# seung-lab/crackle

Measured on AMD Instinct MI355X. Metric: voxels/s encode+decode, 1024x1024x512 uint32; bit-exact .ckl bytes, higher is better.
Workload: dtype u32

## Files before the change

crackle_amd/csrc/ckl_encode.hip:

```cpp
#include "ckl_common.hpp"
#include "ckl_runs.hpp"
#include "ckl_trail.hpp"
#include "ckl_pins_dev.hpp"

#include <algorithm>
#include <atomic>
#include <chrono>
#include <functional>
#include <memory>
#include <mutex>

namespace ckl {

using namespace dev;

template <typename LABEL>
__global__ void __launch_bounds__(kBlock) k_stats(const LABEL* __restrict__ labels, uint64_t voxels, unsigned long long* __restrict__ out ) {
	__shared__ unsigned long long s_max[kWaves], s_pairs[kWaves];
	unsigned long long mx = 0, pairs = 0;
	const uint64_t stride = static_cast<uint64_t>(gridDim.x) * kBlock;
	for (uint64_t i = static_cast<uint64_t>(blockIdx.x) * kBlock + threadIdx.x; i < voxels; i += stride) {
		const LABEL v = labels[i];
		if (static_cast<unsigned long long>(v) > mx) mx = v;
		if (i > 0) pairs += (labels[i - 1] == v);
// ... 1290 lines not shown
	std::vector<uint32_t> code_len;
	uint64_t total = 0;
	bool any_chain = false;
};

inline size_t trail_walk_lds(uint32_t max_special) { return (static_cast<size_t>(max_special) + 256) * 16 + 1024; }

void crack_pass(
	ckl_encoder& e, int64_t sx, int64_t sy, int64_t sz, bool permissible,
	int markov_order, bool hist_only, const std::vector<uint8_t>* model_in,
	std::vector<uint32_t>* hist_out, std::vector<uint8_t>* model_out, CrackResult* result,
	const std::function<void()>& overlap = std::function<void()>(), bool reuse_trail = false
) {
	hipStream_t s = e.stream;
	const uint32_t ns = static_cast<uint32_t>(sz);
	const uint64_t nverts = static_cast<uint64_t>(sx + 1) * (sy + 1);
	e.d_slice_err.ensure(ns);
	const bool prezeroed = e.trail_zeroed && !reuse_trail;
	e.trail_zeroed = false;
	if (prezeroed) CKL_HIP(hipStreamWaitEvent(s, e.ev_prezero, 0));
	if (!reuse_trail && !prezeroed) CKL_HIP(hipMemsetAsync(e.d_slice_err.p, 0, ns * sizeof(uint32_t), s));
	const uint64_t interior = static_cast<uint64_t>(sx > 0 ? sx - 1 : 0) * sy + static_cast<uint64_t>(sx) * (sy > 0 ? sy - 1 : 0);

	std::vector<uint64_t> cbase(ns), sbase(ns), kbase(ns);
	std::vector<uint32_t> ccap(ns), scap(ns), kcap(ns), max_steps(ns);
	std::vector<uint64_t> nbase(ns), cobase(ns), ibase(ns);
	std::vector<uint32_t> ncap(ns), cocap(ns), icap(ns);
	uint64_t ctot = 0, stot = 0, ktot = 0, ntot = 0, cotot = 0, itot = 0;
	uint32_t max_ncap = 0, max_cocap = 0, max_icap = 0, max_special = 0;
	bool any = false;
	for (uint32_t zi = 0; zi < ns; zi++) {
		const uint64_t differ = static_cast<uint64_t>(e.count_v[zi]) + e.count_h[zi];
		const uint64_t E = permissible ? interior - differ : differ;
		any = any || E > 0;
		const uint64_t cc = ((7 * E + 16 + 15) / 16) * 16;
		if (cc > 0xFFFFFFF0ull) throw Error(CKL_ERR_RUNTIME, "crackle_amd: slice has too many crack edges");
		cbase[zi] = ctot; ccap[zi] = static_cast<uint32_t>(cc); ctot += cc;
		max_steps[zi] = static_cast<uint32_t>(E + 1);
		const uint64_t nc = ((static_cast<uint64_t>(e.count_special[zi]) + e.count_corner[zi] + 16) / 16) * 16;
		if (nc >= (1ull << 28)) throw Error(CKL_ERR_RUNTIME, "crackle_amd: slice has too many crack vertices");
		nbase[zi] = ntot; ncap[zi] = static_cast<uint32_t>(nc); ntot += nc;
		cobase[zi] = cotot; cocap[zi] = e.count_corner[zi]; cotot += e.count_corner[zi];
		const uint64_t ic = 7 * nc + 16;
		ibase[zi] = itot; icap[zi] = static_cast<uint32_t>(ic); itot += ic;
		sbase[zi] = stot; scap[zi] = static_cast<uint32_t>(2 * nc + 4); stot += 2 * nc + 4;
		kbase[zi] = ktot; kcap[zi] = static_cast<uint32_t>(nc); ktot += nc;
		max_ncap = std::max<uint32_t>(max_ncap, ncap[zi]);
		max_cocap = std::max<uint32_t>(max_cocap, cocap[zi]);
		max_icap = std::max<uint32_t>(max_icap, icap[zi]);
		max_special = std::max<uint32_t>(max_special, e.count_special[zi]);
	}
	if (result) result->any_chain = any;
	if (g_ht && g_ht->on) {
		uint32_t over = 0;
		for (uint32_t zi = 0; zi < ns; zi++) over += e.count_special[zi] > 3584u;
		fprintf(stderr, "[ckl trail nodes] max special %u, slices above 3584: %u of %u\n", max_special, over, ns);
	}
	HT_MARK("c:caps");
	UploadPacker tables;
	tables.add(e.d_cbase, cbase); tables.add(e.d_ccap, ccap);
	tables.add(e.d_sbase, sbase); tables.add(e.d_scap, scap);
	tables.add(e.d_kbase, kbase); tables.add(e.d_kcap, kcap);
	e.d_cp.ensure(ctot); e.d_fcode.ensure(ctot);
	if (markov_order) e.d_dcode.ensure(ctot);
	e.d_stack_node.ensure(stot); e.d_stack_code.ensure(stot);
	e.d_chain_node.ensure(ktot); e.d_chain_off.ensure(ktot); e.d_chain_clen.ensure(ktot);
	e.d_chain_order.ensure(ktot); e.d_chain_dst.ensure(ktot); e.d_chain_vstart.ensure(ktot);
	e.d_n_chains.ensure(ns); e.d_n_raw.ensure(ns); e.d_n_valid.ensure(ns);
	e.d_payload_len.ensure(ns); e.d_boc_len.ensure(ns);

	const int xw = byte_width(static_cast<uint64_t>(sx) + 1), yw = byte_width(static_cast<uint64_t>(sy) + 1);
	std::vector<uint64_t> pbase(ns), bbase(ns);
	uint64_t ptot = 0, btot = 0;
	for (uint32_t zi = 0; zi < ns; zi++) {
		const uint64_t ncodes = ccap[zi];
		const uint64_t pbytes = markov_order ? (3ull * ncodes + 2 + 7) / 8 : (ncodes + 3) / 4;
		pbase[zi] = ptot; ptot += ((pbytes + 8 + 3) / 4) * 4;
		const uint64_t bbytes = 4 + yw + static_cast<uint64_t>(kcap[zi]) * (yw + 2 * xw);
		bbase[zi] = btot; btot += bbytes;
	}
	tables.add(e.d_pbase, pbase); tables.add(e.d_bbase, bbase);
	tables.add(e.t_nbase, nbase); tables.add(e.t_ncap, ncap);
	tables.add(e.t_cobase, cobase); tables.add(e.t_cocap, cocap);
	tables.add(e.t_ibase, ibase); tables.add(e.t_icap, icap);
	tables.add(e.t_max_steps, max_steps);
	tables.commit(e.d_crack_tables, s, e.uploads_by_kernel ? &e.tables_staging : nullptr);
	HT_MARK("c:tables");
	e.d_payload.ensure(ptot + 8); e.d_boc.ensure(btot + 8);
	e.codes_capacity = ptot + btot;
	if (markov_order) CKL_HIP(hipMemsetAsync(e.d_payload.p, 0, ptot + 8, s));

	FinishArgs fa;
	fa.sx = static_cast<int>(sx); fa.sy = static_cast<int>(sy); fa.xw = xw; fa.yw = yw;
	fa.markov = markov_order ? 1u : 0u;
	fa.cbase = e.d_cbase.p; fa.kbase = e.d_kbase.p;
	fa.n_chains = e.d_n_chains.p; fa.n_raw = e.d_n_raw.p; fa.n_valid = e.d_n_valid.p;
	fa.cp = e.d_cp.p; fa.chain_node = e.d_chain_node.p; fa.chain_off = e.d_chain_off.p; fa.chain_clen = e.d_chain_clen.p;
	fa.chain_order = e.d_chain_order.p; fa.chain_dst = e.d_chain_dst.p; fa.chain_vstart = e.d_chain_vstart.p;
	fa.fcode = e.d_fcode.p; fa.dcode = e.d_dcode.p;
	fa.pbase = e.d_pbase.p; fa.payload = e.d_payload.p; fa.bbase = e.d_bbase.p; fa.boc = e.d_boc.p;
	fa.payload_len = e.d_payload_len.p; fa.boc_len = e.d_boc_len.p;

	unsigned long long* ta_dbg = nullptr;
	size_t trail_lds_used = 0;
	DevBuf<unsigned long long> d_tdbg;
	CKL_HIP(hipEventRecord(e.evk0, s));
	if (!reuse_trail) {
		e.t_counters.ensure(7 * static_cast<size_t>(ns));
		if (!prezeroed) CKL_HIP(hipMemsetAsync(e.t_counters.p, 0, 7 * static_cast<size_t>(ns) * sizeof(uint32_t), s));
		e.t_node_vertex.ensure(ntot); e.t_node_adj.ensure(ntot + 16); e.t_vert2node.ensure(nverts * ns);
		e.t_corner_vertex.ensure(cotot);
		e.t_dart_end.ensure(4 * ntot); e.t_dart_len.ensure(4 * ntot); e.t_dart_minv.ensure(4 * ntot); e.t_dart_minpos.ensure(4 * ntot);
		e.t_dart_codes.ensure(4 * ntot); e.t_dart_inline.ensure(4 * ntot);
		e.t_parent.ensure(ntot); e.t_compmin.ensure(ntot); e.t_starts.ensure(ntot);
		const uint32_t start_words = static_cast<uint32_t>((nverts + 31) / 32);
		e.t_start_bits.ensure(static_cast<size_t>(start_words) * ns);
		if (!prezeroed) CKL_HIP(hipMemsetAsync(e.t_start_bits.p, 0, static_cast<size_t>(start_words) * ns * sizeof(uint32_t), s));
		e.t_items.ensure(itot); e.t_item_off.ensure(itot); e.t_chain_item0.ensure(ktot);
		e.t_events.ensure(itot); e.t_chain_ev0.ensure(ktot); e.t_ev_lnd.ensure(itot); e.t_ev_item.ensure(itot);

		TrailArgs ta;
		ta.adjm = e.d_adjm.p; ta.adjm_stride = e.adjm_stride; ta.mtx2 = e.mtx2; ta.tiles_x = e.tiles_x; ta.tiles_y = e.tiles_y;
		ta.planeV = e.d_planes.p; ta.planeH = e.d_planes.p + e.plane_words * ns; ta.row_words = e.row_words; ta.plane_words = e.plane_words;
		ta.sx = static_cast<uint32_t>(sx); ta.sy = static_cast<uint32_t>(sy); ta.inv = e.graph_permissible ? 0xFFFFFFFFu : 0u;
		ta.sxe = static_cast<uint32_t>(sx + 1); ta.sye = static_cast<uint32_t>(sy + 1); ta.nverts = static_cast<uint32_t>(nverts);
		ta.max_steps = e.t_max_steps.p;
		ta.nbase = e.t_nbase.p; ta.ncap = e.t_ncap.p;
		ta.n_nodes = e.t_counters.p; ta.n_corners = e.t_counters.p + 2 * ns;
		ta.n_starts = e.t_counters.p + 3 * ns; ta.n_items = e.t_counters.p + 4 * ns;
		ta.node_vertex = e.t_node_vertex.p; ta.node_adj = e.t_node_adj.p; ta.vert2node = e.t_vert2node.p;
		ta.cobase = e.t_cobase.p; ta.cocap = e.t_cocap.p; ta.corner_vertex = e.t_corner_vertex.p;
		ta.dart_end = e.t_dart_end.p; ta.dart_len = e.t_dart_len.p; ta.dart_minv = e.t_dart_minv.p; ta.dart_minpos = e.t_dart_minpos.p;
		ta.dart_codes = e.t_dart_codes.p; ta.dart_inline = e.t_dart_inline.p;
		ta.parent = e.t_parent.p; ta.compmin = e.t_compmin.p;
		ta.start_bits = e.t_start_bits.p; ta.start_words = start_words; ta.starts = e.t_starts.p;
		ta.ibase = e.t_ibase.p; ta.icap = e.t_icap.p; ta.items = e.t_items.p; ta.item_off = e.t_item_off.p;
		ta.sbase = e.d_sbase.p; ta.scap = e.d_scap.p; ta.stack_node = e.d_stack_node.p; ta.stack_item = e.d_stack_code.p;
		ta.kbase = e.d_kbase.p; ta.kcap = e.d_kcap.p;
		ta.chain_node = e.d_chain_node.p; ta.chain_item0 = e.t_chain_item0.p; ta.chain_off = e.d_chain_off.p; ta.chain_clen = e.d_chain_clen.p;
		ta.n_chains = e.d_n_chains.p; ta.n_raw = e.d_n_raw.p; ta.n_valid = e.d_n_valid.p;
		ta.cbase = e.d_cbase.p; ta.ccap = e.d_ccap.p; ta.cp = e.d_cp.p; ta.slice_err = e.d_slice_err.p;

		e.last_trail_slices = ns;
		ta.events = e.t_events.p; ta.n_events = e.t_counters.p + 5 * ns; ta.seg_len_sum = e.t_counters.p + 6 * ns; ta.chain_ev0 = e.t_chain_ev0.p; ta.ev_lnd = e.t_ev_lnd.p; ta.ev_item = e.t_ev_item.p;
		ta.dbg = nullptr;
		{ const char* env = getenv("CKL_TRAIL_WALK"); ta.walk_plain = (env && !strcmp(env, "plain")) ? 1u : 0u; ta.walk_no_regs = (env && !strcmp(env, "lds")) ? 1u : 0u; }
		{ const char* env = getenv("CKL_TRAIL_WALK_STACK"); ta.walk_stack_cap = env ? static_cast<uint32_t>(std::max(1, atoi(env))) : 0xFFFFFFFFu; }
		if (kTuning && getenv("CKL_TRAIL_DIAG")) { d_tdbg.ensure(16); CKL_HIP(hipMemsetAsync(d_tdbg.p, 0, 128, s)); ta.dbg = d_tdbg.p; ta_dbg = d_tdbg.p; }
		ta.graph_blocks = e.graph_blocks; ta.blk_special = e.t_blk_special.p; ta.blk_corner = e.t_blk_corner.p;
		int max_lds = 0;
		CKL_HIP(hipDeviceGetAttribute(&max_lds, hipDeviceAttributeMaxSharedMemoryPerBlock, e.device));
		const size_t budget = static_cast<size_t>(max_lds > 1024 ? max_lds - 1024 : 0);
		const uint32_t dart_blocks = (4 * max_ncap + kWalkChunk * kWaves - 1) / (kWalkChunk * kWaves);
		size_t clds = (static_cast<size_t>(max_special) + 1024) * 4;
		if (const char* env = getenv("CKL_TRAIL_LDS")) clds = static_cast<size_t>(std::max(0, atoi(env)));
		clds = (std::min(budget, std::max<size_t>(clds, 1024)) / 16) * 16;
		CKL_HIP(hipFuncSetAttribute(reinterpret_cast<const void*>(&k_trail_components), hipFuncAttributeMaxDynamicSharedMemorySize, static_cast<int>(clds)));
		size_t lds = trail_walk_lds(max_special);
		if (const char* env = getenv("CKL_TRAIL_LDS")) lds = static_cast<size_t>(std::max(0, atoi(env)));
		lds = std::min(budget, std::max<size_t>(lds, 4096));
		lds = (lds / 16) * 16;
		CKL_HIP(hipFuncSetAttribute(reinterpret_cast<const void*>(&k_trail_walk), hipFuncAttributeMaxDynamicSharedMemorySize, static_cast<int>(lds)));
		trail_lds_used = lds;
		HT_MARK("c:setup");

		ta.z0 = 0;
		fa.z0 = 0;
		if (any) {
			hipLaunchKernelGGL(k_trail_nodes, dim3(e.graph_blocks, ns), dim3(kBlock), 0, s, ta);
			hipLaunchKernelGGL(k_trail_segments, dim3(dart_blocks, ns), dim3(kBlock), 0, s, ta);
			if (max_cocap) hipLaunchKernelGGL(k_trail_loops, dim3((max_cocap + kBlock - 1) / kBlock, ns), dim3(kBlock), 0, s, ta);
			hipLaunchKernelGGL(k_trail_components, dim3(ns), dim3(kCompBlock), clds, s, ta, static_cast<uint32_t>(clds));
		}
		CKL_HIP(hipEventRecord(e.evd0, s));
		hipLaunchKernelGGL(k_trail_walk, dim3(ns), dim3(kWave), lds, s, ta, static_cast<uint32_t>(lds));
		CKL_HIP(hipEventRecord(e.evd1, s));
		hipLaunchKernelGGL(k_trail_items, dim3(ns), dim3(kItemsBlock), 0, s, ta);
		hipLaunchKernelGGL(k_trail_offsets, dim3(ns), dim3(kBlock), 0, s, ta);
		hipLaunchKernelGGL(k_trail_expand, dim3((max_icap + kExpandChunk * kWaves - 1) / (kExpandChunk * kWaves), ns), dim3(kBlock), 0, s, ta);
		hipLaunchKernelGGL(k_finish, dim3(ns), dim3(kFinishBlock), 0, s, fa);
	}
	CKL_HIP(hipEventRecord(e.evk1, s));
	HT_MARK("c:enqueue");
	if (kTuning && getenv("CKL_TRAIL_DIAG")) {
		std::vector<uint32_t> c = download(e.t_counters.p, 5 * static_cast<size_t>(ns), s);
		double m[5] = { 0 };
		for (int k = 0; k < 5; k++) for (uint32_t zi = 0; zi < ns; zi++) m[k] += static_cast<double>(c[static_cast<size_t>(k) * ns + zi]) / ns;
		double sp = 0, co = 0;
		for (uint32_t zi = 0; zi < ns; zi++) { sp += static_cast<double>(e.count_special[zi]) / ns; co += static_cast<double>(e.count_corner[zi]) / ns; }
		if (ta_dbg) {
			std::vector<unsigned long long> g = download(ta_dbg, 16, s);
			if (g[11]) fprintf(stderr, "[ckl trail diag, k_trail_walk] mean cycles per slice: table fill=%.0f fill + walk=%.0f\n", static_cast<double>(g[6]) / g[11], static_cast<double>(g[7]) / g[11]);
			if (g[11]) fprintf(stderr, "[ckl trail diag, k_trail_walk] slices=%llu iterations/slice=%.0f cycles/iteration=%.0f clock=%.2f GHz (cycles / 100 MHz ticks)\n",
				g[11], static_cast<double>(g[8]) / g[11], g[8] ? static_cast<double>(g[9]) / g[8] : 0.0, g[10] ? static_cast<double>(g[9]) / (g[10] * 10.0) : 0.0);
			fprintf(stderr, "[ckl trail diag, k_trail_components, mean cycles per slice] union=%.0f component minima=%.0f starts/splits=%.0f bitmap scan=%.0f\n",
				static_cast<double>(g[12]) / ns, static_cast<double>(g[13]) / ns, static_cast<double>(g[14]) / ns, static_cast<double>(g[15]) / ns);
			fprintf(stderr, "[ckl trail diag, k_trail_segments] waves=%llu iterations/wave mean=%.1f max=%llu cycles/wave mean=%.0f max=%llu cycles/iteration=%.0f active lanes/iteration=%.1f\n",
				g[4], g[4] ? static_cast<double>(g[0]) / g[4] : 0.0, g[1], g[4] ? static_cast<double>(g[2]) / g[4] : 0.0, g[3],
				g[0] ? static_cast<double>(g[2]) / g[0] : 0.0, g[0] ? static_cast<double>(g[5]) / g[0] : 0.0);
		}
		fprintf(stderr, "[ckl trail diag] max degree-1/3/4 vertices of a slice=%u, k_trail_walk LDS=%zu bytes\n", max_special, trail_lds_used);
		fprintf(stderr, "[ckl trail diag, mean per slice] degree-1/3/4 vertices=%.0f corners=%.0f nodes=%.0f starts=%.0f items=%.0f\n", sp, co, m[0], m[3], m[4]);
	}

	const bool early_tail = !markov_order && result != nullptr;
	auto enqueue_tail = [&]() {
		e.d_out_off.ensure(ns);
		e.d_code_report.ensure(static_cast<size_t>(ns) + 3);
		e.d_codes_out.ensure(e.codes_capacity + 8);
		hipLaunchKernelGGL(k_code_offsets, dim3(1), dim3(kBlock), 0, s, e.d_boc_len.p, e.d_payload_len.p, e.d_slice_err.p, ns, e.d_out_off.p, e.d_code_report.p);
		hipLaunchKernelGGL(k_gather_codes, dim3(ns), dim3(kBlock), 0, s, e.d_boc.p, e.d_bbase.p, e.d_boc_len.p,
			e.d_payload.p, e.d_pbase.p, e.d_payload_len.p, e.d_out_off.p, e.d_codes_out.p);
	};
	if (early_tail) enqueue_tail();
	if (overlap) overlap();
	HT_MARK("c:overlap");


	if (markov_order) {
		std::vector<uint8_t> model;
		if (model_in) {
			model = *model_in;
		}
		else {
			const size_t rows = static_cast<size_t>(1) << (2 * markov_order);
			e.d_hist.ensure(rows * 4);
			CKL_HIP(hipMemsetAsync(e.d_hist.p, 0, rows * 4 * sizeof(uint32_t), s));
			const uint32_t hist_lds = (rows * 4 <= 16384) ? static_cast<uint32_t>(rows * 4) : 0u;
			if (hist_lds * 4 > 48 * 1024) CKL_HIP(hipFuncSetAttribute(reinterpret_cast<const void*>(&k_markov_hist), hipFuncAttributeMaxDynamicSharedMemorySize, static_cast<int>(hist_lds * 4)));
			hipLaunchKernelGGL(k_markov_hist, dim3(ns), dim3(kBlock), hist_lds * sizeof(uint32_t), s, e.d_dcode.p, e.d_cbase.p, e.d_n_valid.p, markov_order, e.d_hist.p, hist_lds);
			std::vector<uint32_t> hist = download(e.d_hist.p, rows * 4, s);
			if (hist_out) *hist_out = hist;
			if (hist_only) {
				std::vector<uint32_t> errs = download(e.d_slice_err.p, ns, s);
				for (uint32_t zi = 0; zi < ns; zi++) if (errs[zi]) throw Error(CKL_ERR_RUNTIME, "crackle_amd: crack walk scratch overflow on z=" + std::to_string(zi));
				return;
			}
			model = markov_stats_to_model(hist.data(), rows);
		}
		if (model_out) *model_out = model;
		upload(e.d_model, model, s);
		hipLaunchKernelGGL(k_markov_pack, dim3(ns), dim3(kBlock), 0, s, e.d_dcode.p, e.d_cbase.p, e.d_n_valid.p, markov_order,
			e.d_model.p, e.d_pbase.p, e.d_payload.p, e.d_payload_len.p);
	}
	if (!result) { CKL_HIP(hipStreamSynchronize(s)); return; }

	if (!early_tail) enqueue_tail();
	HT_MARK("c:finish_enq");
	std::vector<uint32_t> report = download(e.d_code_report.p, static_cast<size_t>(ns) + 3, s);
	HT_MARK("c:finish_wait");
	if (report[ns + 2]) {
		std::vector<uint32_t> errs = download(e.d_slice_err.p, ns, s);
		for (uint32_t zi = 0; zi < ns; zi++) {
			if (errs[zi]) throw Error(CKL_ERR_RUNTIME, "crackle_amd: crack walk scratch overflow on z=" + std::to_string(zi));
		}
	}
	result->code_len.assign(report.begin(), report.begin() + ns);
	const uint64_t otot = static_cast<uint64_t>(report[ns]) | (static_cast<uint64_t>(report[ns + 1]) << 32);
	result->total = otot;
}

struct FlatResult {
	std::vector<uint32_t> ncomp;
	std::vector<uint32_t> crcs;
	uint64_t total = 0;
};

void ensure_geom_table(ckl_encoder& e, uint64_t sxy) {
	if (e.g_table_pixels == sxy && e.d_G.p) return;
	hipStream_t s = e.stream2;
	const uint32_t npx = static_cast<uint32_t>(sxy);
	const uint32_t B = 1024, nblk = npx / B + 1;
	std::vector<uint32_t> g_base(B), blk_g(nblk), blk_x(nblk);
	const uint32_t X = gf_xpow(32);
	g_base[0] = 0;
	for (uint32_t i = 1; i < B; i++) g_base[i] = gf_mul(X, g_base[i - 1] ^ 0x80000000u);
	const uint32_t gB = gf_mul(X, g_base[B - 1] ^ 0x80000000u);
	const uint32_t XB = gf_xpow(32ull * B);
	blk_g[0] = 0; blk_x[0] = 0x80000000u;
	for (uint32_t k = 1; k < nblk; k++) {
		blk_g[k] = blk_g[k - 1] ^ gf_mul(blk_x[k - 1], gB);
		blk_x[k] = gf_mul(blk_x[k - 1], XB);
	}
	DevBuf<uint32_t> t_base, t_g, t_x;
	upload(t_base, g_base, s); upload(t_g, blk_g, s); upload(t_x, blk_x, s);
	e.d_G.ensure(static_cast<size_t>(npx) + 1);
	hipLaunchKernelGGL(k_build_geom_table, dim3(npx / kBlock + 1), dim3(kBlock), 0, s, t_base.p, t_g.p, t_x.p, npx, e.d_G.p);
	CKL_HIP(hipStreamSynchronize(s));
	e.g_table_pixels = sxy;
}

void flat_enqueue(ckl_encoder& e, int64_t sx, int64_t sy, int64_t sz) {
	hipStream_t s = e.stream2;
	const uint32_t ns = static_cast<uint32_t>(sz);
	const uint64_t sxy = static_cast<uint64_t>(sx) * sy;
	ensure_geom_table(e, sxy);

	std::vector<uint64_t>& rbase = e.h_rbase;
	std::vector<uint32_t>& rcap = e.h_rcap;
	rbase.assign(ns, 0); rcap.assign(ns, 0);
	uint64_t rtot = 0;
	uint32_t max_rcap = 0;
	for (uint32_t zi = 0; zi < ns; zi++) {
		const uint64_t runs = static_cast<uint64_t>(sy) + e.count_v[zi];
		rbase[zi] = rtot; rcap[zi] = static_cast<uint32_t>(runs); rtot += runs;
		max_rcap = std::max<uint32_t>(max_rcap, static_cast<uint32_t>(runs));
	}
// ... 1395 lines not shown
```

crackle_amd/csrc/ckl_trail.hpp:

```cpp
#pragma once

#include "ckl_device.hpp"

namespace ckl {
namespace dev {

constexpr uint32_t kTrailTileShift = 5, kTrailTileDim = 32;
__device__ __forceinline__ uint32_t mt_index(uint32_t mx, uint32_t my, uint32_t mtx2) {
	return (((my >> 1) * mtx2 + (mx >> 1)) << 2) | ((my & 1u) << 1) | (mx & 1u);
}
struct MicroTile {
	uint4 lo, hi;
	uint32_t mx, my;
	__device__ __forceinline__ bool holds(uint32_t x, uint32_t y) const { return (x >> 3) == mx && (y >> 3) == my; }
	__device__ __forceinline__ uint32_t nib(uint32_t x, uint32_t y) const {
		const uint32_t r = y & 7u;
		const uint32_t a0 = (r & 1u) ? lo.y : lo.x, a1 = (r & 1u) ? lo.w : lo.z, a2 = (r & 1u) ? hi.y : hi.x, a3 = (r & 1u) ? hi.w : hi.z;
		const uint32_t b0 = (r & 2u) ? a1 : a0, b1 = (r & 2u) ? a3 : a2;
		return (((r & 4u) ? b1 : b0) >> ((x & 7u) * 4u)) & 15u;
	}
};

enum : uint32_t { TRAIL_ERR_CAPACITY = 1u };
constexpr uint32_t kDartNone = 0xFFFFFFFFu;
// ... 323 lines not shown
		cq.z = __builtin_amdgcn_alignbit(cq.w, cq.z, 2);
		cq.w = (cq.w >> 2) | (trail_code(kk) << 30);
	};
	unsigned long long dbg_iter = 0, dbg_lane = 0;
	const unsigned long long dbg_t0 = a.dbg ? __builtin_amdgcn_s_memtime() : 0ull;
	for (;;) {
		if (a.dbg) { dbg_iter++; dbg_lane += __popcll(__ballot(active)); }
		const unsigned long long need = __ballot(!active);
		const bool refill = next < range_end && (__popcll(need) >= kWalkRefill || need == ~0ull);
		const uint32_t cand = next + static_cast<uint32_t>(__popcll(need & lt_mask));
		const bool take = refill && !active && cand < range_end;
		uint32_t r_adj = 0, r_v0 = 0;
		if (take) { r_adj = a.node_adj[nb + (cand >> 2)]; r_v0 = a.node_vertex[nb + (cand >> 2)]; }
		if (active && !c.holds(x, y)) mt_load(c, adjm, x, y, a.mtx2);
		for (int it = 0; it < kWalkAhead; it++) {
			const bool go = active && c.holds(x, y);
			if (!__ballot(go)) break;
			if (go) {
				const uint32_t w = y * a.sxe + x;
				const uint32_t arr = k ^ 1u;
				if (w < minv) { minv = w; minpos = (steps << 2) | arr; }
				const uint32_t nib = c.nib(x, y);
				bool fin = false;
				if (__popc(nib) != 2) fin = true;
				else if (steps >= cap) { err = TRAIL_ERR_CAPACITY; fin = true; }
				else { k = __ffs(nib & ~(1u << arr)) - 1; push_code(k); trail_step(x, y, k); steps++; }
				if (fin) {
					res[d - range_begin] = make_uint4((w << 2) | arr, steps, minv, minpos);
					res_codes[d - range_begin] = cq;
					active = false;
				}
			}
		}
		if (take && ((r_adj >> (cand & 3u)) & 1u)) {
			d = cand; k = cand & 3u;
			y = r_v0 / a.sxe; x = r_v0 - y * a.sxe;
			minv = r_v0; minpos = 0;
			push_code(k);
			trail_step(x, y, k);
			steps = 1;
			active = true;
		}
		if (refill) next += static_cast<uint32_t>(__popcll(need));
		if (!__ballot(active) && next >= range_end) break;
	}
	if (a.dbg && lane == 0) {
		const unsigned long long cyc = __builtin_amdgcn_s_memtime() - dbg_t0;
		atomicAdd(a.dbg + 0, dbg_iter); atomicMax(a.dbg + 1, dbg_iter);
		atomicAdd(a.dbg + 2, cyc); atomicMax(a.dbg + 3, cyc);
		atomicAdd(a.dbg + 4, 1ull); atomicAdd(a.dbg + 5, dbg_lane);
	}
	const uint64_t db = nb * 4u + range_begin;
	uint32_t len_sum = 0;
	for (uint32_t i = lane; i < range_end - range_begin; i += kWave) {
		const uint4 r = res[i];
		a.dart_end[db + i] = r.x == kDartNone ? kDartNone : ((v2n[r.x >> 2] << 2) | (r.x & 3u));
		a.dart_len[db + i] = r.y;
		a.dart_minv[db + i] = r.z;
		a.dart_minpos[db + i] = r.w;
		const uint4 q = res_codes[i];
		const bool whole = r.x != kDartNone && r.y >= 1u && r.y <= kInlineCodes;
		uint4 o = make_uint4(0, 0, 0, 0);
		if (whole) {
			const uint32_t sh = 128u - 2u * r.y, w = sh >> 5, b = sh & 31u;
			const uint32_t v[5] = { q.x, q.y, q.z, q.w, 0u };
			auto word = [&](uint32_t t) -> uint32_t { return t == 0 ? v[0] : t == 1 ? v[1] : t == 2 ? v[2] : t == 3 ? v[3] : 0u; };
			auto pick = [&](uint32_t t) -> uint32_t { return __builtin_amdgcn_alignbit(word(t + w + 1u), word(t + w), b); };
			o = make_uint4(pick(0), pick(1), pick(2), pick(3));
			(void)v;
		}
		a.dart_codes[db + i] = o;
		a.dart_inline[db + i] = whole ? 1u : 0u;
		len_sum += r.x == kDartNone ? 0u : r.y;
	}
	len_sum = wave_sum(len_sum);
	if (lane == 0 && len_sum) atomicAdd(a.seg_len_sum + zi, len_sum);
	if (err) atomicOr(a.slice_err + zi, err);
}

static __global__ void __launch_bounds__(kBlock) k_trail_loops(TrailArgs a) {
	const uint32_t zi = blockIdx.y + a.z0;
	if (a.seg_len_sum[zi] == 2u * (a.max_steps[zi] - 1u)) return;
	const uint32_t ci = blockIdx.x * kBlock + threadIdx.x;
	const uint32_t nc = min(a.n_corners[zi], a.cocap[zi]);
	const uint4* adjm = a.adjm + zi * a.adjm_stride;
	const uint32_t cap = a.max_steps[zi];
	bool active = ci < nc;
	const uint32_t v0 = active ? a.corner_vertex[a.cobase[zi] + ci] : 0u;
	uint32_t y = v0 / a.sxe, x = v0 - y * a.sxe;
	uint32_t k = 0, steps = 1;
	trail_step(x, y, k);
	bool loop = false;
	MicroTile c;
	c.lo = c.hi = make_uint4(0, 0, 0, 0); c.mx = c.my = 0xFFFFFFFFu;
	while (__ballot(active)) {
		if (active && !c.holds(x, y)) mt_load(c, adjm, x, y, a.mtx2);
		for (int it = 0; it < kWalkAhead; it++) {
			const bool go = active && c.holds(x, y);
			if (!__ballot(go)) break;
			if (go) {
				const uint32_t w = y * a.sxe + x;
				const uint32_t nib = c.nib(x, y);
				if (w == v0) { loop = true; active = false; }
				else if (w < v0 || __popc(nib) != 2 || steps >= cap) active = false;
				else { k = __ffs(nib & ~(1u << (k ^ 1u))) - 1; trail_step(x, y, k); steps++; }
			}
		}
	}
	if (!loop) return;
	const uint32_t j = atomicAdd(a.n_nodes + zi, 1u);
	if (j >= a.ncap[zi]) { atomicOr(a.slice_err + zi, TRAIL_ERR_CAPACITY); return; }
	const uint64_t nb = a.nbase[zi];
	a.node_vertex[nb + j] = v0;
	a.node_adj[nb + j] = 5u;
	a.vert2node[static_cast<uint64_t>(zi) * a.nverts + v0] = j;
	const uint64_t db = (nb + j) * 4u;
	for (uint32_t q = 0; q < 4; q++) { a.dart_end[db + q] = kDartNone; a.dart_len[db + q] = 0; a.dart_minv[db + q] = v0; a.dart_minpos[db + q] = 0; a.dart_inline[db + q] = 0; }
	a.dart_end[db + 0] = (j << 2) | 2u; a.dart_len[db + 0] = steps;
	a.dart_end[db + 2] = (j << 2) | 0u; a.dart_len[db + 2] = steps;
}

template <bool LDS>
__device__ __forceinline__ uint32_t tuf_load(uint32_t* L, uint32_t i) {
	if (LDS) return __hip_atomic_load(L + i, __ATOMIC_RELAXED, __HIP_MEMORY_SCOPE_WORKGROUP);
	return __hip_atomic_load(L + i, __ATOMIC_RELAXED, __HIP_MEMORY_SCOPE_AGENT);
}
template <bool LDS>
__device__ __forceinline__ uint32_t tuf_find(uint32_t* L, uint32_t a) {
	uint32_t p = tuf_load<LDS>(L, a);
	while (p != a) {
		const uint32_t gp = tuf_load<LDS>(L, p);
		if (gp != p) atomicMin(L + a, gp);
		a = p;
		p = gp;
	}
	return a;
}
template <bool LDS>
__device__ __forceinline__ void tuf_unite(uint32_t* L, uint32_t a, uint32_t b) {
	for (;;) {
		a = tuf_find<LDS>(L, a);
		b = tuf_find<LDS>(L, b);
		if (a == b) return;
		if (a > b) { const uint32_t t = a; a = b; b = t; }
		const uint32_t old = atomicMin(L + b, a);
		if (old == b) return;
		b = old;
	}
}

constexpr uint32_t kStartList = 2048;
constexpr int kCompBlock = 256;

template <bool LDS>
__device__ __forceinline__ void trail_components_slice(const TrailArgs& a, uint32_t zi, uint32_t* parent, uint32_t nn, uint32_t* s_scan, uint32_t* s_nstart) {
	const uint64_t nb = a.nbase[zi];
	uint32_t* start_tmp = a.items + a.ibase[zi];
	unsigned long long dg_t = a.dbg ? __builtin_amdgcn_s_memtime() : 0ull;
	auto stamp = [&](int slot) { if (a.dbg && threadIdx.x == 0) { const unsigned long long now = __builtin_amdgcn_s_memtime(); atomicAdd(a.dbg + slot, now - dg_t); dg_t = now; } };
	const uint32_t* dart_end = a.dart_end + nb * 4u;
	unsigned long long* compmin = a.compmin + nb;
	for (uint32_t j = threadIdx.x; j < nn; j += kCompBlock) { parent[j] = j; compmin[j] = ~0ull; }
	__syncthreads();
	if (!LDS) __threadfence();
	constexpr uint32_t kUniteBatch = 8;
	for (uint32_t d0 = threadIdx.x; d0 < nn * 4u; d0 += kCompBlock * kUniteBatch) {
		uint32_t e[kUniteBatch];
#pragma unroll
		for (uint32_t k = 0; k < kUniteBatch; k++) {
			const uint32_t d = d0 + k * kCompBlock;
			e[k] = d < nn * 4u ? dart_end[d] : kDartNone;
		}
#pragma unroll
		for (uint32_t k = 0; k < kUniteBatch; k++) {
			if (e[k] == kDartNone) continue;
			const uint32_t j = (d0 + k * kCompBlock) >> 2, j2 = e[k] >> 2;
			if (j < j2 && j2 < nn) tuf_unite<LDS>(parent, j, j2);
		}
	}
	__syncthreads();
	if (!LDS) __threadfence();
	stamp(12);
	for (uint32_t j0 = 0; j0 < nn; j0 += kCompBlock) {
		const uint32_t j = j0 + threadIdx.x;
		uint32_t root = 0xFFFFFFFFu;
		unsigned long long val = ~0ull;
		if (j < nn) {
			const uint4 e4 = *reinterpret_cast<const uint4*>(dart_end + j * 4u);
			const uint4 m4 = *reinterpret_cast<const uint4*>(a.dart_minv + nb * 4u + j * 4u);
			const uint32_t ee[4] = { e4.x, e4.y, e4.z, e4.w }, mm[4] = { m4.x, m4.y, m4.z, m4.w };
#pragma unroll
			for (uint32_t k = 0; k < 4u; k++) {
				if (ee[k] == kDartNone) continue;
				const unsigned long long v = (static_cast<unsigned long long>(mm[k]) << 32) | (j * 4u + k);
				val = v < val ? v : val;
			}
			if (val != ~0ull) root = tuf_find<LDS>(parent, j);
		}
		unsigned long long todo = __ballot(root != 0xFFFFFFFFu);
		while (todo) {
			const int first = __ffsll(static_cast<long long>(todo)) - 1;
			const uint32_t r0 = __shfl(root, first, kWave);
			const bool mine = (root == r0);
			unsigned long long v = mine ? val : ~0ull;
#pragma unroll
			for (int s = kWave / 2; s >= 1; s >>= 1) {
				const unsigned long long o = __shfl_xor(v, s, kWave);
				v = o < v ? o : v;
			}
			if ((threadIdx.x & (kWave - 1)) == first) atomicMin(compmin + r0, v);
			todo &= ~__ballot(mine);
		}
	}
	__syncthreads();
	__threadfence();
	stamp(13);
	uint32_t* bits = a.start_bits + static_cast<uint64_t>(zi) * a.start_words;
	for (uint32_t j = threadIdx.x; j < nn; j += kCompBlock) {
		if (tuf_load<LDS>(parent, j) != j) continue;
		const unsigned long long m = __hip_atomic_load(compmin + j, __ATOMIC_RELAXED, __HIP_MEMORY_SCOPE_AGENT);
		if (m == ~0ull) continue;
		const uint32_t minv = static_cast<uint32_t>(m >> 32);
		const uint32_t d = static_cast<uint32_t>(m);
		atomicOr(bits + (minv >> 5), 1u << (minv & 31u));
		{
			const uint32_t slot = atomicAdd(s_nstart, 1u);
			if (slot < kStartList) start_tmp[slot] = minv;
		}
		const uint64_t db = nb * 4u;
		const uint32_t len = a.dart_len[db + d];
		const uint32_t pos = a.dart_minpos[db + d] >> 2, arr = a.dart_minpos[db + d] & 3u;
		if (pos == 0 || pos == len) continue;
		const uint32_t s = atomicAdd(a.n_nodes + zi, 1u);
		if (s >= a.ncap[zi]) { atomicOr(a.slice_err + zi, TRAIL_ERR_CAPACITY); continue; }
		a.node_vertex[nb + s] = minv;
		a.node_adj[nb + s] = 5u;
		a.vert2node[static_cast<uint64_t>(zi) * a.nverts + minv] = s;
		const uint32_t d2 = a.dart_end[db + d];
		const uint32_t other = arr ^ 2u;
		for (uint32_t q = 0; q < 4; q++) { a.dart_end[db + s * 4u + q] = kDartNone; a.dart_len[db + s * 4u + q] = 0; a.dart_inline[db + s * 4u + q] = 0; }
		a.dart_end[db + d] = (s << 2) | arr;        a.dart_len[db + d] = pos;
		a.dart_end[db + d2] = (s << 2) | other;     a.dart_len[db + d2] = len - pos;
		a.dart_end[db + s * 4u + arr] = d;          a.dart_len[db + s * 4u + arr] = pos;
		a.dart_end[db + s * 4u + other] = d2;       a.dart_len[db + s * 4u + other] = len - pos;
	}
	__syncthreads();
	__threadfence();
	stamp(14);
	uint32_t* starts = a.starts + nb;
	const uint32_t cap = a.kcap[zi];
	const uint32_t n_listed = *s_nstart;
	if (n_listed <= kStartList) {
		for (uint32_t i = threadIdx.x; i < n_listed; i += kCompBlock) {
			const uint32_t v = __hip_atomic_load(start_tmp + i, __ATOMIC_RELAXED, __HIP_MEMORY_SCOPE_AGENT);
			uint32_t rank = 0;
			for (uint32_t q = 0; q < n_listed; q++) rank += __hip_atomic_load(start_tmp + q, __ATOMIC_RELAXED, __HIP_MEMORY_SCOPE_AGENT) < v ? 1u : 0u;
			if (rank < cap) starts[rank] = v;
			else atomicOr(a.slice_err + zi, TRAIL_ERR_CAPACITY);
		}
		if (threadIdx.x == 0) a.n_starts[zi] = n_listed < cap ? n_listed : cap;
		stamp(15);
		return;
	}
	constexpr uint32_t kPer = 8;
	uint32_t carry = 0, err = 0;
	for (uint32_t w0 = 0; w0 < a.start_words; w0 += kCompBlock * kPer) {
		uint32_t b[kPer], cnt = 0;
#pragma unroll
		for (uint32_t q = 0; q < kPer; q++) {
			const uint32_t wi = w0 + threadIdx.x * kPer + q;
			b[q] = wi < a.start_words ? __hip_atomic_load(bits + wi, __ATOMIC_RELAXED, __HIP_MEMORY_SCOPE_AGENT) : 0u;
			cnt += __popc(b[q]);
		}
		uint32_t v[1] = { cnt }, tot[1];
		block_excl_add<1, kCompBlock / kWave>(v, tot, s_scan);
		uint32_t o = carry + v[0];
#pragma unroll
		for (uint32_t q = 0; q < kPer; q++) {
			const uint32_t wi = w0 + threadIdx.x * kPer + q;
			for (uint32_t m = b[q]; m; m &= m - 1u) {
				if (o < cap) starts[o] = wi * 32u + (__ffs(m) - 1);
				else err = TRAIL_ERR_CAPACITY;
				o++;
			}
		}
		carry += tot[0];
	}
	if (threadIdx.x == 0) a.n_starts[zi] = carry < cap ? carry : cap;
	if (err) atomicOr(a.slice_err + zi, err);
	stamp(15);
}

static __global__ void __launch_bounds__(kCompBlock) k_trail_components(TrailArgs a, uint32_t lds_bytes) {
	extern __shared__ uint32_t s_trail[];
	__shared__ uint32_t s_scan[kCompBlock / kWave];
	__shared__ uint32_t s_nstart;
	const uint32_t zi = blockIdx.x + a.z0;
	const uint32_t nn = min(a.n_nodes[zi], a.ncap[zi]);
	if (threadIdx.x == 0) s_nstart = 0;
	__syncthreads();
	if (nn * 4u <= lds_bytes) trail_components_slice<true>(a, zi, s_trail, nn, s_scan, &s_nstart);
	else trail_components_slice<false>(a, zi, a.parent + a.nbase[zi], nn, s_scan, &s_nstart);
}

enum : uint32_t { TCODE_UP = 0, TCODE_RIGHT = 1, TCODE_DOWN = 2, TCODE_LEFT = 3, TCODE_NONE = 0xFE };

struct TrailTabLds {
	uint8_t* adj;
	unsigned long long* end4;
	__device__ __forceinline__ void load(uint32_t j, uint32_t& av, uint32_t& e_lo, uint32_t& e_hi) const {
		const uint32_t a0 = adj[j];
		const unsigned long long e = end4[j];
		av = __builtin_amdgcn_readfirstlane(a0);
		e_lo = __builtin_amdgcn_readfirstlane(static_cast<uint32_t>(e));
		e_hi = __builtin_amdgcn_readfirstlane(static_cast<uint32_t>(e >> 32));
	}
	__device__ __forceinline__ uint32_t pick(uint32_t e_lo, uint32_t e_hi, uint32_t k) const {
		const uint32_t w = (k & 2u) ? e_hi : e_lo;
		return (w >> ((k & 1u) * 16u)) & 0xFFFFu;
	}
	__device__ __forceinline__ void set_adj(uint32_t j, uint32_t v) const { adj[j] = static_cast<uint8_t>(v); }
};
struct TrailTabGlobal {
	uint8_t* adj;
	const uint32_t* end;
	__device__ __forceinline__ void load(uint32_t j, uint32_t& av, uint32_t& e_lo, uint32_t& e_hi) const {
		const uint32_t* w = reinterpret_cast<const uint32_t*>(reinterpret_cast<uintptr_t>(adj + j) & ~static_cast<uintptr_t>(3));
		const uint32_t sh = static_cast<uint32_t>(reinterpret_cast<uintptr_t>(adj + j) & 3u) * 8u;
		av = (__builtin_amdgcn_readfirstlane(__hip_atomic_load(w, __ATOMIC_RELAXED, __HIP_MEMORY_SCOPE_AGENT)) >> sh) & 0xFFu;
		e_lo = j; e_hi = 0;
	}
	__device__ __forceinline__ uint32_t pick(uint32_t e_lo, uint32_t e_hi, uint32_t k) const { return __builtin_amdgcn_readfirstlane(end[e_lo * 4u + k]); }
	__device__ __forceinline__ void set_adj(uint32_t j, uint32_t v) const {
		uint32_t* w = reinterpret_cast<uint32_t*>(reinterpret_cast<uintptr_t>(adj + j) & ~static_cast<uintptr_t>(3));
		const uint32_t sh = static_cast<uint32_t>(reinterpret_cast<uintptr_t>(adj + j) & 3u) * 8u;
		const uint32_t old = __hip_atomic_load(w, __ATOMIC_RELAXED, __HIP_MEMORY_SCOPE_AGENT);
		__hip_atomic_store(w, (old & ~(0xFFu << sh)) | ((v & 0xFFu) << sh), __ATOMIC_RELAXED, __HIP_MEMORY_SCOPE_AGENT);
	}
};

constexpr uint32_t kEvSeg = 0u << 30, kEvBseg = 1u << 30, kEvDead = 2u << 30, kEvEnd = 3u << 30, kEvMask = 3u << 30;
constexpr uint32_t kEvFormatAddr12 = 1u << 31;
constexpr uint32_t kEvWalkWide = 1u << 30;

template <typename TAB>
__device__ __forceinline__ void trail_walk_slice(
	const TrailArgs& a, uint32_t zi, const TAB& tab, uint2* s_stack2, uint32_t lds_slots
) {
	const uint64_t nb = a.nbase[zi];
	const uint32_t* starts = a.starts + nb;
	const uint32_t n_starts = a.n_starts[zi];
	uint32_t* ev = a.events + a.ibase[zi];
	const uint32_t ecap = a.icap[zi];
	uint32_t* st_node = a.stack_node + a.sbase[zi];
	uint32_t* st_ev = a.stack_item + a.sbase[zi];
	const uint32_t scap = a.scap[zi];
	uint32_t* ch_node = a.chain_node + a.kbase[zi];
	uint32_t* ch_ev0 = a.chain_ev0 + a.kbase[zi];
	const uint32_t kcap = a.kcap[zi];
	const uint32_t* vert2node = a.vert2node + static_cast<uint64_t>(zi) * a.nverts;
	const uint32_t cap1 = lds_slots - 1u;

	uint32_t ne = 0, nch = 0, err = 0;
	const unsigned long long dbg_t0 = (kTuning && a.dbg) ? __builtin_amdgcn_s_memtime() : 0ull;
	const unsigned long long dbg_r0 = (kTuning && a.dbg) ? __builtin_amdgcn_s_memrealtime() : 0ull;
	for (uint32_t si = 0; si < n_starts && !err; si++) {
		const uint32_t sv = __builtin_amdgcn_readfirstlane(starts[si]);
		uint32_t j = __builtin_amdgcn_readfirstlane(vert2node[sv]);
		if (nch < kcap) { ch_node[nch] = sv; ch_ev0[nch] = ne; }
		else err |= TRAIL_ERR_CAPACITY;
		nch++;
		uint32_t sp = 0, pend = 0;
		for (;;) {
			if (ne + 2u > ecap) { err |= TRAIL_ERR_CAPACITY; break; }
			uint32_t av_raw, e_lo, e_hi;
			tab.load(j, av_raw, e_lo, e_hi);
			const uint2 top = s_stack2[sp < cap1 ? sp : cap1];
			const uint32_t av = av_raw & ~pend;
			if (av == 0) {
				tab.set_adj(j, 0u);
				if (sp == 0) { ev[ne] = kEvEnd; ne++; break; }
				uint32_t pj = __builtin_amdgcn_readfirstlane(top.x), pev = __builtin_amdgcn_readfirstlane(top.y);
				if (sp > cap1) {
					pj = __builtin_amdgcn_readfirstlane(__hip_atomic_load(st_node + sp - 1u, __ATOMIC_RELAXED, __HIP_MEMORY_SCOPE_AGENT));
					pev = __builtin_amdgcn_readfirstlane(__hip_atomic_load(st_ev + sp - 1u, __ATOMIC_RELAXED, __HIP_MEMORY_SCOPE_AGENT));
				}
				ev[ne] = kEvDead | pev;
				ne++; sp--; pend = 0; j = pj;
				continue;
			}
			const uint32_t k = __ffs(av) - 1;
			const uint32_t rest = av & ~(1u << k);
			tab.set_adj(j, rest);
			const uint32_t e = tab.pick(e_lo, e_hi, k);
			const bool multi = rest != 0;
			if (multi && sp >= cap1) {
				if (sp < scap) { st_node[sp] = j; st_ev[sp] = ne; }
				else err |= TRAIL_ERR_CAPACITY;
			}
			s_stack2[(multi && sp < cap1) ? sp + 1u : 0u] = make_uint2(j, ne);
			ev[ne] = (multi ? kEvBseg : kEvSeg) | (j * 4u + k);
			ne++;
			sp += multi ? 1u : 0u;
			pend = 1u << (e & 3u);
			j = e >> 2;
		}
	}
	if (kTuning && a.dbg) {
		atomicAdd(a.dbg + 8, static_cast<unsigned long long>(ne));
		atomicAdd(a.dbg + 9, __builtin_amdgcn_s_memtime() - dbg_t0);
		atomicAdd(a.dbg + 10, __builtin_amdgcn_s_memrealtime() - dbg_r0);
		atomicAdd(a.dbg + 11, 1ull);
	}
	a.n_events[zi] = ne < ecap ? ne : ecap;
	a.n_chains[zi] = nch < kcap ? nch : kcap;
	if (err) atomicOr(a.slice_err + zi, err);
}

__device__ __forceinline__ uint32_t trail_walk_chain_fast(
	uint32_t j_addr, uint32_t& ev_off, uint32_t& ev_left, uint32_t stack_base, uint32_t max_depth, uint32_t* ev
) {
	uint32_t status, off = ev_off, left = ev_left;
	const uint32_t top0 = stack_base - 4u;
	const uint32_t ev_lo = __builtin_amdgcn_readfirstlane(static_cast<uint32_t>(reinterpret_cast<uintptr_t>(ev)));
	const uint32_t ev_hi = __builtin_amdgcn_readfirstlane(static_cast<uint32_t>(reinterpret_cast<uintptr_t>(ev) >> 32));
	j_addr = __builtin_amdgcn_readfirstlane(j_addr);
	max_depth = __builtin_amdgcn_readfirstlane(max_depth);
	asm volatile(
		"s_setprio 3\n"
		"s_mov_b32 s40, %[j]\n"
		"s_mov_b32 s41, 0\n"
		"s_mov_b32 s42, 0\n"
		"v_readfirstlane_b32 s43, %[left]\n"
		"s_mov_b32 s52, %[evlo]\n"
		"s_mov_b32 s53, %[evhi]\n"
		"s_mov_b32 s54, %[maxd]\n"
		"v_mov_b32 v29, %[off]\n"
		"v_mov_b32 v25, %[top]\n"
		"1:\n"
		"v_mov_b32 v20, s40\n"
		"ds_read2_b32 v[32:33], v20 offset1:1\n"
		"ds_read_b32 v34, v20 offset:8\n"
		"ds_read_b32 v26, v25\n"
		"s_sub_u32 s43, s43, 1\n"
		"s_cbranch_scc1 8f\n"
		"s_waitcnt lgkmcnt(0)\n"
		"v_readfirstlane_b32 s46, v32\n"
		"v_readfirstlane_b32 s44, v33\n"
		"v_readfirstlane_b32 s45, v34\n"
		"s_andn2_b32 s46, s46, s41\n"
		"s_cbranch_scc0 4f\n"
		"s_ff1_i32_b32 s47, s46\n"
		"s_bitset0_b32 s46, s47\n"
		"v_mov_b32 v21, s46\n"
		"ds_write_b32 v20, v21\n"
// ... 856 lines not shown
```

Measured before the change: 152.2 billion.

## Keep per-node component minimum in LDS and fuse its computation with union pass

The per-node minimum dart key is now computed while the union-find unite pass reads each node's four dart ends, so the second pass no longer reloads dart_end and dart_minv. When the slice fits, the compmin array lives in LDS next to the parent array, with a larger LDS request (12 bytes per node), and several device-wide fences become block-scope or are removed. It also hoists the dart_len, dart_minpos and dart_end loads ahead of the atomics. The cost is more LDS per block, which may lower occupancy, and an extra template variant.

```diff
diff --git a/crackle_amd/csrc/ckl_encode.hip b/crackle_amd/csrc/ckl_encode.hip
--- a/crackle_amd/csrc/ckl_encode.hip
+++ b/crackle_amd/csrc/ckl_encode.hip
@@ -1466,7 +1466,7 @@
 		CKL_HIP(hipDeviceGetAttribute(&max_lds, hipDeviceAttributeMaxSharedMemoryPerBlock, e.device));
 		const size_t budget = static_cast<size_t>(max_lds > 1024 ? max_lds - 1024 : 0);
 		const uint32_t dart_blocks = (4 * max_ncap + kWalkChunk * kWaves - 1) / (kWalkChunk * kWaves);
-		size_t clds = (static_cast<size_t>(max_special) + 1024) * 4;
+		size_t clds = (static_cast<size_t>(max_special) + 1024) * 12;
 		if (const char* env = getenv("CKL_TRAIL_LDS")) clds = static_cast<size_t>(std::max(0, atoi(env)));
 		clds = (std::min(budget, std::max<size_t>(clds, 1024)) / 16) * 16;
 		CKL_HIP(hipFuncSetAttribute(reinterpret_cast<const void*>(&k_trail_components), hipFuncAttributeMaxDynamicSharedMemorySize, static_cast<int>(clds)));
diff --git a/crackle_amd/csrc/ckl_trail.hpp b/crackle_amd/csrc/ckl_trail.hpp
--- a/crackle_amd/csrc/ckl_trail.hpp
+++ b/crackle_amd/csrc/ckl_trail.hpp
@@ -499,50 +499,67 @@
 constexpr uint32_t kStartList = 2048;
 constexpr int kCompBlock = 256;
 
-template <bool LDS>
-__device__ __forceinline__ void trail_components_slice(const TrailArgs& a, uint32_t zi, uint32_t* parent, uint32_t nn, uint32_t* s_scan, uint32_t* s_nstart) {
+template <bool LDS, bool CMLDS>
+__device__ __forceinline__ void trail_components_slice(const TrailArgs& a, uint32_t zi, uint32_t* parent, unsigned long long* compmin, uint32_t nn, uint32_t* s_scan, uint32_t* s_nstart) {
 	const uint64_t nb = a.nbase[zi];
 	uint32_t* start_tmp = a.items + a.ibase[zi];
 	unsigned long long dg_t = a.dbg ? __builtin_amdgcn_s_memtime() : 0ull;
 	auto stamp = [&](int slot) { if (a.dbg && threadIdx.x == 0) { const unsigned long long now = __builtin_amdgcn_s_memtime(); atomicAdd(a.dbg + slot, now - dg_t); dg_t = now; } };
 	const uint32_t* dart_end = a.dart_end + nb * 4u;
-	unsigned long long* compmin = a.compmin + nb;
-	for (uint32_t j = threadIdx.x; j < nn; j += kCompBlock) { parent[j] = j; compmin[j] = ~0ull; }
+	auto cm_load = [&](uint32_t j) -> unsigned long long {
+		if (CMLDS) return __hip_atomic_load(compmin + j, __ATOMIC_RELAXED, __HIP_MEMORY_SCOPE_WORKGROUP);
+		return __hip_atomic_load(compmin + j, __ATOMIC_RELAXED, __HIP_MEMORY_SCOPE_AGENT);
+	};
+	for (uint32_t j = threadIdx.x; j < nn; j += kCompBlock) parent[j] = j;
 	__syncthreads();
 	if (!LDS) __threadfence();
-	constexpr uint32_t kUniteBatch = 8;
-	for (uint32_t d0 = threadIdx.x; d0 < nn * 4u; d0 += kCompBlock * kUniteBatch) {
-		uint32_t e[kUniteBatch];
-#pragma unroll
-		for (uint32_t k = 0; k < kUniteBatch; k++) {
-			const uint32_t d = d0 + k * kCompBlock;
-			e[k] = d < nn * 4u ? dart_end[d] : kDartNone;
-		}
-#pragma unroll
-		for (uint32_t k = 0; k < kUniteBatch; k++) {
-			if (e[k] == kDartNone) continue;
-			const uint32_t j = (d0 + k * kCompBlock) >> 2, j2 = e[k] >> 2;
-			if (j < j2 && j2 < nn) tuf_unite<LDS>(parent, j, j2);
+	constexpr uint32_t kNodeBatch = 4;
+	for (uint32_t j0 = threadIdx.x; j0 < nn; j0 += kCompBlock * kNodeBatch) {
+		uint4 e4[kNodeBatch], m4[kNodeBatch];
+#pragma unroll
+		for (uint32_t k = 0; k < kNodeBatch; k++) {
+			const uint32_t j = j0 + k * kCompBlock;
+			e4[k] = make_uint4(kDartNone, kDartNone, kDartNone, kDartNone);
+			m4[k] = make_uint4(0u, 0u, 0u, 0u);
+			if (j < nn) {
+				e4[k] = *reinterpret_cast<const uint4*>(dart_end + j * 4u);
+				m4[k] = *reinterpret_cast<const uint4*>(a.dart_minv + nb * 4u + j * 4u);
+			}
+		}
+#pragma unroll
+		for (uint32_t k = 0; k < kNodeBatch; k++) {
+			const uint32_t j = j0 + k * kCompBlock;
+			if (j >= nn) continue;
+			const uint32_t ee[4] = { e4[k].x, e4[k].y, e4[k].z, e4[k].w }, mm[4] = { m4[k].x, m4[k].y, m4[k].z, m4[k].w };
+			unsigned long long val = ~0ull;
+#pragma unroll
+			for (uint32_t q = 0; q < 4u; q++) {
+				if (ee[q] == kDartNone) continue;
+				const unsigned long long v = (static_cast<unsigned long long>(mm[q]) << 32) | (j * 4u + q);
+				val = v < val ? v : val;
+			}
+			compmin[j] = val;
+#pragma unroll
+			for (uint32_t q = 0; q < 4u; q++) {
+				if (ee[q] == kDartNone) continue;
+				const uint32_t j2 = ee[q] >> 2;
+				if (j < j2 && j2 < nn) tuf_unite<LDS>(parent, j, j2);
+			}
 		}
 	}
 	__syncthreads();
-	if (!LDS) __threadfence();
+	if (!LDS || !CMLDS) __threadfence();
 	stamp(12);
 	for (uint32_t j0 = 0; j0 < nn; j0 += kCompBlock) {
 		const uint32_t j = j0 + threadIdx.x;
 		uint32_t root = 0xFFFFFFFFu;
 		unsigned long long val = ~0ull;
 		if (j < nn) {
-			const uint4 e4 = *reinterpret_cast<const uint4*>(dart_end + j * 4u);
-			const uint4 m4 = *reinterpret_cast<const uint4*>(a.dart_minv + nb * 4u + j * 4u);
-			const uint32_t ee[4] = { e4.x, e4.y, e4.z, e4.w }, mm[4] = { m4.x, m4.y, m4.z, m4.w };
-#pragma unroll
-			for (uint32_t k = 0; k < 4u; k++) {
-				if (ee[k] == kDartNone) continue;
-				const unsigned long long v = (static_cast<unsigned long long>(mm[k]) << 32) | (j * 4u + k);
-				val = v < val ? v : val;
-			}
-			if (val != ~0ull) root = tuf_find<LDS>(parent, j);
+			val = cm_load(j);
+			if (val != ~0ull) {
+				root = tuf_find<LDS>(parent, j);
+				if (root == j) root = 0xFFFFFFFFu;
+			}
 		}
 		unsigned long long todo = __ballot(root != 0xFFFFFFFFu);
 		while (todo) {
@@ -560,30 +577,31 @@
 		}
 	}
 	__syncthreads();
-	__threadfence();
+	if (!CMLDS) __threadfence();
 	stamp(13);
 	uint32_t* bits = a.start_bits + static_cast<uint64_t>(zi) * a.start_words;
 	for (uint32_t j = threadIdx.x; j < nn; j += kCompBlock) {
 		if (tuf_load<LDS>(parent, j) != j) continue;
-		const unsigned long long m = __hip_atomic_load(compmin + j, __ATOMIC_RELAXED, __HIP_MEMORY_SCOPE_AGENT);
+		const unsigned long long m = cm_load(j);
 		if (m == ~0ull) continue;
 		const uint32_t minv = static_cast<uint32_t>(m >> 32);
 		const uint32_t d = static_cast<uint32_t>(m);
+		const uint64_t db = nb * 4u;
+		const uint32_t len = a.dart_len[db + d];
+		const uint32_t mp = a.dart_minpos[db + d];
+		const uint32_t d2 = a.dart_end[db + d];
 		atomicOr(bits + (minv >> 5), 1u << (minv & 31u));
 		{
 			const uint32_t slot = atomicAdd(s_nstart, 1u);
 			if (slot < kStartList) start_tmp[slot] = minv;
 		}
-		const uint64_t db = nb * 4u;
-		const uint32_t len = a.dart_len[db + d];
-		const uint32_t pos = a.dart_minpos[db + d] >> 2, arr = a.dart_minpos[db + d] & 3u;
+		const uint32_t pos = mp >> 2, arr = mp & 3u;
 		if (pos == 0 || pos == len) continue;
 		const uint32_t s = atomicAdd(a.n_nodes + zi, 1u);
 		if (s >= a.ncap[zi]) { atomicOr(a.slice_err + zi, TRAIL_ERR_CAPACITY); continue; }
 		a.node_vertex[nb + s] = minv;
 		a.node_adj[nb + s] = 5u;
 		a.vert2node[static_cast<uint64_t>(zi) * a.nverts + minv] = s;
-		const uint32_t d2 = a.dart_end[db + d];
 		const uint32_t other = arr ^ 2u;
 		for (uint32_t q = 0; q < 4; q++) { a.dart_end[db + s * 4u + q] = kDartNone; a.dart_len[db + s * 4u + q] = 0; a.dart_inline[db + s * 4u + q] = 0; }
 		a.dart_end[db + d] = (s << 2) | arr;        a.dart_len[db + d] = pos;
@@ -592,7 +610,7 @@
 		a.dart_end[db + s * 4u + other] = d2;       a.dart_len[db + s * 4u + other] = len - pos;
 	}
 	__syncthreads();
-	__threadfence();
+	if (LDS && CMLDS) __threadfence_block(); else __threadfence();
 	stamp(14);
 	uint32_t* starts = a.starts + nb;
 	const uint32_t cap = a.kcap[zi];
@@ -639,15 +657,16 @@
 }
 
 static __global__ void __launch_bounds__(kCompBlock) k_trail_components(TrailArgs a, uint32_t lds_bytes) {
-	extern __shared__ uint32_t s_trail[];
+	extern __shared__ unsigned long long s_comp[];
 	__shared__ uint32_t s_scan[kCompBlock / kWave];
 	__shared__ uint32_t s_nstart;
 	const uint32_t zi = blockIdx.x + a.z0;
 	const uint32_t nn = min(a.n_nodes[zi], a.ncap[zi]);
 	if (threadIdx.x == 0) s_nstart = 0;
 	__syncthreads();
-	if (nn * 4u <= lds_bytes) trail_components_slice<true>(a, zi, s_trail, nn, s_scan, &s_nstart);
-	else trail_components_slice<false>(a, zi, a.parent + a.nbase[zi], nn, s_scan, &s_nstart);
+	if (static_cast<uint64_t>(nn) * 12u <= lds_bytes) trail_components_slice<true, true>(a, zi, reinterpret_cast<uint32_t*>(s_comp + nn), s_comp, nn, s_scan, &s_nstart);
+	else if (static_cast<uint64_t>(nn) * 4u <= lds_bytes) trail_components_slice<true, false>(a, zi, reinterpret_cast<uint32_t*>(s_comp), a.compmin + a.nbase[zi], nn, s_scan, &s_nstart);
+	else trail_components_slice<false, false>(a, zi, a.parent + a.nbase[zi], a.compmin + a.nbase[zi], nn, s_scan, &s_nstart);
 }
 
 enum : uint32_t { TCODE_UP = 0, TCODE_RIGHT = 1, TCODE_DOWN = 2, TCODE_LEFT = 3, TCODE_NONE = 0xFE };
```

Result: faster. 155.7 billion, median of 6 (+2.3%).
